# szemenyeim/RoboCupVision

Measured on AMD Instinct MI355X. Metric: training images/sec, ROBO-UNet 640x480 bs=32/GPU, higher is better.
Workload: dtype f32; 1 GPU; robo_unet_640x480_bs32; per_gpu_batch=32, global_batch=32, height=480, width=640, step=fwd+CE/argmax+bwd+L1+Adam (train.py:43-74), parallelism=dp1, launch=eager (one rcv_run per pass)

## Files before the change

robocupvision_amd/csrc/conv_bf3.hip:

```cpp
#include <type_traits>
#include "conv_bf3_stage.h"
#include "conv_epilogue.h"

constexpr int C3_PITCH = 192;
constexpr int C3_NU = 13;
constexpr int C3_COT = 64;

template <int WN, bool TWO>
__global__ __launch_bounds__(512) void conv_bf3_kernel(const ConvArgs a) {
  constexpr int WM = 2;
  extern __shared__ __attribute__((aligned(16))) char smem_c3[];
  const int npix = a.IH * a.IW;
  const int xbytes = a.xl_floats * 4;
  float* red = reinterpret_cast<float*>(smem_c3 + 2 * xbytes);
  const bool producer = threadIdx.x >= 256;
  const int tid = producer ? (int)threadIdx.x - 256 : (int)threadIdx.x;
  const TileInfo ti = decode_tile<KIND_GATHER>(a, xcd_remap(blockIdx.x, a.total_tiles), C3_COT);
  const int nchunks = a.nchunks;
  const bool do_stage = !(a.flags & RCV_F_DBG_NOSTAGE), do_mfma = !(a.flags & RCV_F_DBG_NOMFMA);

  if (producer) {
    auto stage = [&](int c, char* buf) { bf3_conv_stage<32, C3_NU, TWO>(a, ti, buf, a.Cin, 32 * c, tid, npix); };
    if (do_stage) stage(0, smem_c3);
    __syncthreads();
    for (int c = 0; c < nchunks; ++c) {
      if (c + 1 < nchunks && do_stage) stage(c + 1, smem_c3 + ((c + 1) & 1) * xbytes);
      __syncthreads();
    }
    if (a.stats != RCV_STATS_NONE) __syncthreads();
    return;
  }

  const int lane = tid & 63, wave = tid >> 6;
  const int wave_m = wave >> 1, wave_n = wave & 1;
  const int l15 = lane & 15, l4 = lane >> 4;
  f32x4 acc[WM][WN];
#pragma unroll
  for (int m = 0; m < WM; ++m)
#pragma unroll
    for (int n = 0; n < WN; ++n) acc[m][n] = (f32x4){0.f, 0.f, 0.f, 0.f};
  int pixoff[WN];
#pragma unroll
  for (int n = 0; n < WN; ++n) {
    const int p = (wave_n * WN + n) * 16 + l15;
    int ty = fd_div(p, a.fdWt), tx = p - ty * a.Wt;
    if (ty >= a.R) { ty = 0; tx = 0; }
    pixoff[n] = (ty * a.IW + tx) * C3_PITCH + l4 * 16;
  }
  const char* wb[WM];
#pragma unroll
  for (int m = 0; m < WM; ++m) {
    int co = ti.co0 + (wave_m * WM + m) * 16 + l15;
    if (co >= a.CoutP) co = a.CoutP - 1;
    wb[m] = reinterpret_cast<const char*>(a.w) + (size_t)co * 64 + l4 * 16;
  }
  const size_t wstep = (size_t)a.CoutP * 64;
  const size_t wplane = 9 * (size_t)nchunks * wstep;
  bf16x8 A[3][WM][3];
  auto load_a = [&](int tap, int c, bf16x8 (&dst)[WM][3]) {
    if (c >= nchunks) { c = nchunks - 1; }
    const size_t o = (size_t)(tap * nchunks + c) * wstep;
#pragma unroll
    for (int m = 0; m < WM; ++m)
#pragma unroll
      for (int pl = 0; pl < 3; ++pl) dst[m][pl] = *reinterpret_cast<const bf16x8*>(wb[m] + pl * wplane + o);
  };
  load_a(0, 0, A[0]);
  load_a(1, 0, A[1]);
  load_a(2, 0, A[2]);
  __syncthreads();
  for (int c = 0; c < nchunks; ++c) {
    const char* xb = smem_c3 + (c & 1) * xbytes;
    if (do_mfma)
#pragma unroll
    for (int tap = 0; tap < 9; ++tap) {
      const int tapoff = ((tap / 3) * a.IW + (tap % 3)) * C3_PITCH;
      const bf16x8 (&Ac)[WM][3] = A[tap % 3];
      bf16x8 B[2][3];
      auto load_b = [&](int n, bf16x8 (&dst)[3]) {
        const char* pb = xb + pixoff[n] + tapoff;
#pragma unroll
        for (int pl = 0; pl < 3; ++pl) dst[pl] = *reinterpret_cast<const bf16x8*>(pb + pl * 64);
      };
      load_b(0, B[0]);
#pragma unroll
      for (int n = 0; n < WN; ++n) {
        if (n + 1 < WN) load_b(n + 1, B[(n + 1) & 1]);
#pragma unroll
        for (int e = 0; e < 6; ++e)
#pragma unroll
          for (int m = 0; m < WM; ++m) acc[m][n] = __builtin_amdgcn_mfma_f32_16x16x32_bf16(Ac[m][BF3_TA[e]], B[n & 1][BF3_TB[e]], acc[m][n], 0, 0, 0);
        if (n + 1 < WN) {
#pragma unroll
          for (int e = 0; e < 3; ++e) {
            __builtin_amdgcn_sched_group_barrier(0x008, 1, 0);
            __builtin_amdgcn_sched_group_barrier(0x100, 1, 0);
          }
        }
        __builtin_amdgcn_sched_barrier(0);
      }
      {
        int t3 = tap + 3, c3 = c;
        if (t3 >= 9) { t3 -= 9; c3 += 1; }
        if (!(a.flags & RCV_F_DBG_NOSKIP)) load_a(t3, c3, A[tap % 3]);
      }
    }
    __syncthreads();
  }
  if (!(a.flags & RCV_F_DBG_NOEPI)) conv_epilogue<WM, WN, 2, 2, KIND_GATHER, 5>(a, ti, acc, red, tid);
  else if (a.stats != RCV_STATS_NONE) __syncthreads();
}

template <int WN, bool TWO>
__global__ __launch_bounds__(512) void conv2_bf3_kernel(const ConvArgs a) {
  constexpr int WM = 2, CH = 16, PITCH = 6 * CH, NKS = 5;
  extern __shared__ __attribute__((aligned(16))) char smem_c3[];
  const int npix = a.IH * a.IW;
  const int xbytes = a.xl_floats * 4;
  float* red = reinterpret_cast<float*>(smem_c3 + 2 * xbytes);
  const bool producer = threadIdx.x >= 256;
  const int tid = producer ? (int)threadIdx.x - 256 : (int)threadIdx.x;
  const TileInfo ti = decode_tile<KIND_GATHER>(a, xcd_remap(blockIdx.x, a.total_tiles), C3_COT);
  const int nchunks = a.nchunks;

  if (producer) {
    auto stage = [&](int c, char* buf) { bf3_conv_stage<CH, C3_NU, TWO>(a, ti, buf, a.Cin, CH * c, tid, npix); };
    stage(0, smem_c3);
    __syncthreads();
    for (int c = 0; c < nchunks; ++c) {
      if (c + 1 < nchunks) stage(c + 1, smem_c3 + ((c + 1) & 1) * xbytes);
      __syncthreads();
    }
    if (a.stats != RCV_STATS_NONE) __syncthreads();
// ... 93 lines not shown
    const int slots = 2 * WN * 16;
    for (int TW = 4; TW <= Wo && TW <= 64; ++TW) {
      int TH = slots / TW;
      if (TH > Ho) TH = Ho;
      if (TH < 1) continue;
      TH = ceil_div(Ho, ceil_div(Ho, TH));
      const int IH = (TH - 1) * S + 3, IW = (TW - 1) * S + 3;
      if (IH * IW > C3_NU * per_pass || IW >= 65536) continue;
      const size_t lds = 2 * (size_t)round_up(IH * IW * pitch, 16) + 2 * 2 * C3_COT * sizeof(float) * 2;
      if (lds > (size_t)h->max_lds) continue;
      const long tiles = (long)N * ceil_div(Ho, TH) * ceil_div(Wo, TW) * n_co;
      const long rounds = ceil_div((int)tiles, h->num_cus);
      const double cost = (double)rounds * (slots + 64) * (1.0 + 0.02 * (double)(IH * IW) / (TH * TW * S * S));
      if (cost < best) {
        best = cost; found = true;
        g->WN = WN; g->TH = TH; g->TW = TW; g->IH = IH; g->IW = IW; g->tiles_x = ceil_div(Wo, TW); g->tiles_y = ceil_div(Ho, TH);
        g->n_co_tiles = n_co; g->total = (int)tiles; g->lds = lds;
      }
    }
  }
  return found;
}

bool conv_bf3_wanted(const rcv_handle* h, const rcv_op* op) {
  if (RCV_ENV("RCV_NO_BF3") || (op->flags & RCV_F_MFMA_FP32)) return false;
  const int N = op->i[RCV_I_N], H = op->i[RCV_I_H], W = op->i[RCV_I_W], Cin = op->i[RCV_I_CIN], Cout = op->i[RCV_I_COUT];
  const int S = op->i[RCV_I_STRIDE];
  if (op->kind != RCV_OP_CONV || (S != 1 && S != 2) || op->i[RCV_I_DIL] != 1) return false;
  if (op->i[RCV_I_INMODE] == RCV_LOAD_NCHW || Cout % 4 || Cout < 64) return false;
  if (S == 1 ? (Cin % 32 || Cin < 64) : (Cin % 16 || Cin < 32 || RCV_ENV("RCV_NO_BF3S2") != nullptr)) return false;
  if (S == 2 && !RCV_ENV("RCV_BF3S2_ALL")) {
    const int m = op->i[RCV_I_INMODE];
    if (m == RCV_LOAD_GRAD_ENC || m == RCV_LOAD_GRAD_DEC) return false;
  }
  if ((long long)N * H * W * Cin >= (1ll << 31)) return false;
  if (RCV_ENV("RCV_BF3_FWD")) {
    const int m = op->i[RCV_I_INMODE];
    if (m == RCV_LOAD_GRAD_ENC || m == RCV_LOAD_GRAD_DEC) return false;
  }
  C3Geom g;
  if (!c3_geometry(h, op, &g)) return false;
  return (long)g.total * 4 >= (long)h->num_cus * 3;
}

bool conv_bf3_supported(const rcv_handle* h, const rcv_op* op, int kind) {
  return kind == KIND_GATHER && ((op->i[RCV_I_AUX0] == 3 && op->i[RCV_I_STRIDE] == 1) || (op->i[RCV_I_AUX0] == 5 && op->i[RCV_I_STRIDE] == 2));
}

int conv_bf3_plan(const rcv_handle* h, const rcv_op* op, ConvPlan* pl) {
  const int Cin = op->i[RCV_I_CIN], Cout = op->i[RCV_I_COUT];
  const int S = op->i[RCV_I_STRIDE];
  RCV_CHECK_ARG(op->kind == RCV_OP_CONV && (S == 1 || S == 2) && op->i[RCV_I_DIL] == 1 && Cin % (S == 1 ? 32 : 16) == 0 && Cout % 4 == 0 &&
                    op->i[RCV_I_INMODE] != RCV_LOAD_NCHW && !(op->flags & RCV_F_MFMA_FP32),
                "split-bf16 conv: needs dilation 1, Cin %% 32 == 0 (stride 1) or %% 16 (stride 2), an NHWC input (got s%d d%d Cin %d Cout %d)", S,
                op->i[RCV_I_DIL], Cin, Cout);
  C3Geom g;
  RCV_CHECK_ARG(c3_geometry(h, op, &g), "split-bf16 conv: no tile fits %dx%d", op->i[RCV_I_HO], op->i[RCV_I_WO]);
  pl->kind = KIND_GATHER; pl->narrow = 0; pl->dma = 0; pl->first = 0; pl->wino = 0; pl->small = 0; pl->bf3 = 1;
  pl->CK = S == 1 ? 32 : 16; pl->CoutV = Cout; pl->CoutP = round_up(Cout, 16);
  pl->R = g.TH; pl->Wt = g.TW; pl->IH = g.IH; pl->IW = g.IW; pl->tiles_x = g.tiles_x; pl->tiles_y = g.tiles_y;
  pl->n_co_tiles = g.n_co_tiles; pl->n_phases = 1; pl->total_tiles = g.total; pl->grid = g.total;
  pl->WN = g.WN; pl->WM = 2;
  pl->xl_floats = round_up(g.IH * g.IW * (S == 1 ? C3_PITCH : C3_PITCH / 2), 16) / 4; pl->wl_floats = 0;
  pl->lds = g.lds;
  return RCV_OK;
}

int conv_bf3_launch(const ConvPlan& pl, const ConvArgs& a, hipStream_t s) {
  const bool two = a.in_mode == RCV_LOAD_GRAD_ENC || a.in_mode == RCV_LOAD_GRAD_DEC;
  if (a.stride == 2) return two ? conv_launch_with_lds<conv2_bf3_kernel<5, true>>(pl, a, s) : conv_launch_with_lds<conv2_bf3_kernel<5, false>>(pl, a, s);
  if (pl.WN == 10) return two ? conv_launch_with_lds<conv_bf3_kernel<10, true>>(pl, a, s) : conv_launch_with_lds<conv_bf3_kernel<10, false>>(pl, a, s);
  return two ? conv_launch_with_lds<conv_bf3_kernel<5, true>>(pl, a, s) : conv_launch_with_lds<conv_bf3_kernel<5, false>>(pl, a, s);
}
```

robocupvision_amd/csrc/conv_bf3_stage.h:

```cpp
#pragma once
#include "conv_common.h"
#include "split_bf16.h"

template <int NU, bool TWO>
struct Bf3ConvRegs {
  float4 x[NU], ax[TWO ? NU : 1];
  bool ok[NU];
};

template <int CH, int NU, bool TWO>
__device__ __forceinline__ void bf3_conv_load(Bf3ConvRegs<NU, TWO>& r, const ConvArgs& a, const TileInfo& ti, int C, int c0, int tid, int npix) {
  constexpr int Q = CH / 4, PP = 256 / Q;
  const int q = tid % Q, lp = tid / Q;
#pragma unroll
  for (int u = 0; u < NU; ++u) {
    const int pix = u * PP + lp;
    const int iy = fd_div(pix, a.fdIW), ix = pix - iy * a.IW;
    const int gy = ti.oy0 + iy, gx = ti.ox0 + ix;
    r.ok[u] = pix < npix && (unsigned)gy < (unsigned)a.H && (unsigned)gx < (unsigned)a.W;
    const uint32_t o = r.ok[u] ? (uint32_t)(((ti.n * a.H + gy) * a.W + gx) * C + c0 + 4 * q) : 0u;
    r.x[u] = ld4(a.in + o);
    if (TWO) r.ax[u] = ld4(a.in_aux + o);
  }
}
template <int MODE, int CH, int NU, bool TWO>
__device__ __forceinline__ void bf3_conv_store(const Bf3ConvRegs<NU, TWO>& r, const ConvArgs& a, char* img, int C, int c0, int tid, int npix) {
  constexpr int Q = CH / 4, PP = 256 / Q;
  const int q = tid % Q, lp = tid / Q;
  float4 k[5];
  if (MODE != RCV_LOAD_PLAIN) {
#pragma unroll
    for (int j = 0; j < 5; ++j) k[j] = ld4(a.in_c + (size_t)j * C + c0 + 4 * q);
  }
#pragma unroll
  for (int u = 0; u < NU; ++u) {
    const int pix = u * PP + lp;
    float4 v = xform4<MODE>(r.x[u], r.ax[TWO ? u : 0], k);
    if (!r.ok[u]) v = make_float4(0.f, 0.f, 0.f, 0.f);
    if (pix < npix) {
      const Bf3Tri lo = bf3_split2(v.x, v.y), hi = bf3_split2(v.z, v.w);
      char* d = img + pix * (6 * CH) + 8 * q;
      *reinterpret_cast<uint2*>(d) = make_uint2(lo.h, hi.h);
      *reinterpret_cast<uint2*>(d + 2 * CH) = make_uint2(lo.m, hi.m);
      *reinterpret_cast<uint2*>(d + 4 * CH) = make_uint2(lo.l, hi.l);
    }
  }
}

template <int CH, int NU, bool TWO>
__device__ __forceinline__ void bf3_conv_stage(const ConvArgs& a, const TileInfo& ti, char* img, int C, int c0, int tid, int npix) {
  Bf3ConvRegs<NU, TWO> r;
  bf3_conv_load<CH, NU, TWO>(r, a, ti, C, c0, tid, npix);
  with_load_mode<TWO>(a.in_mode, [&](auto mode) { bf3_conv_store<mode(), CH, NU, TWO>(r, a, img, C, c0, tid, npix); });
}
```

robocupvision_amd/csrc/conv_common.h:

```cpp
#pragma once
#include "load_xform.h"

enum { KIND_GATHER = 0, KIND_TPHASE = 1, KIND_TMERGED = 2, KIND_TALL = 3 };

struct ConvArgs {
  const float* in;
  const float* in_aux;
  const float* in_c;
  const float* w;
  const float* bias;
  float* out;
  const float* resid;
  const float* epi_aux;
  const float* epi_c;
  float* part;
  int N, H, W, Cin, Cout, Ho, Wo;
  int CinP, CoutP, CoutV;
  int stride, dil;
  int R, Wt, tiles_x, tiles_y, IH, IW;
  int n_pix_tiles, n_co_tiles, n_sub, total_tiles, nchunks;
  int in_mode, stats;
  uint32_t flags;
  int wl_floats, xl_floats;
  int xpitch;
// ... 24 lines not shown
  ti.x0 = tx_i * a.Wt;
  ti.co0 = co_tile * COT;
  ti.py = phase >> 1;
  ti.px = phase & 1;
  if (KIND == KIND_GATHER) { ti.oy0 = ti.y0 * a.stride - a.dil; ti.ox0 = ti.x0 * a.stride - a.dil; }
  else { ti.oy0 = ti.y0; ti.ox0 = ti.x0; }
  return ti;
}

struct ConvPlan {
  int kind, tile, CK, R, Wt, tiles_x, tiles_y, IH, IW;
  int CoutV, CoutP, n_co_tiles, n_phases, total_tiles, grid;
  size_t lds;
  int wl_floats, xl_floats;
  int narrow;
  int dma;
  int xk;
  int WM, WN, XMAX;
  int first;
  int dev;
  int wino;
  int bf3;
  int small;
};

template <auto KERN>
static int conv_launch_with_lds(const ConvPlan& pl, const ConvArgs& a, hipStream_t s) {
  return rcv_launch_with_lds<KERN>(a, dim3(pl.grid), pl.lds, pl.dev, s);
}

static inline int conv_xpitch(int CK, int pixel_stride) {
  if (const char* ev = RCV_ENV("RCV_XPITCH_PAD")) return CK + atoi(ev);
  return pixel_stride == 1 ? CK + 2 : CK + 1;
}

static inline void tile_halo(int kind, int R, int Wt, int s, int d, int* IH, int* IW) {
  if (kind == KIND_GATHER) { *IH = (R - 1) * s + 2 * d + 1; *IW = (Wt - 1) * s + 2 * d + 1; }
  else { *IH = R + 1; *IW = Wt + 1; }
}

bool conv_wino_supported(const rcv_handle* h, const rcv_op* op, int kind);
bool conv_wino_wanted(const rcv_handle* h, const rcv_op* op, bool force);
int conv_wino_plan(const rcv_handle* h, const rcv_op* op, ConvPlan* pl);
int conv_wino_launch(const ConvPlan& pl, const ConvArgs& a, hipStream_t s);

bool conv_bf3_wanted(const rcv_handle* h, const rcv_op* op);
bool conv_bf3_supported(const rcv_handle* h, const rcv_op* op, int kind);
int conv_bf3_plan(const rcv_handle* h, const rcv_op* op, ConvPlan* pl);
int conv_bf3_launch(const ConvPlan& pl, const ConvArgs& a, hipStream_t s);

bool convn_bf3_wanted(const rcv_handle* h, const rcv_op* op);
// ... 16 lines not shown
```

robocupvision_amd/csrc/conv_epilogue.h:

```cpp
#pragma once
#include "conv_common.h"

template <int WM, int WN, int WAVES_M, int WAVES_N, int KIND, int EB = (WM == 1 ? WN : 0)>
__device__ __forceinline__ void conv_epilogue_tile(const ConvArgs& a, const TileInfo& ti, f32x4 (&acc)[WM][WN], float (&s1)[WM][4], float (&s2)[WM][4], int tid) {
  const int lane = tid & 63, wave = tid >> 6;
  const int wave_m = wave / WAVES_N, wave_n = wave % WAVES_N;
  const int l15 = lane & 15, l4 = lane >> 4;
#pragma unroll
    for (int m = 0; m < WM; ++m) {
      const int cov = ti.co0 + (wave_m * WM + m) * 16 + 4 * l4;
      int co = cov, py = ti.py, pxx = ti.px;
      if (KIND == KIND_TMERGED) { const int ph = cov / a.Cout; co = cov - ph * a.Cout; py = ph >> 1; pxx = ph & 1; }
      const bool co_ok = cov < a.CoutV;
      float4 bias = make_float4(0.f, 0.f, 0.f, 0.f);
      float4 e0 = bias, e1 = bias, mu = bias;
      if (co_ok) {
        if (a.flags & RCV_F_BIAS) bias = ld4(a.bias + co);
        if (a.stats == RCV_STATS_BWD_DEC) { e0 = ld4(a.epi_c + co); e1 = ld4(a.epi_c + a.Cout + co); }
        if (a.stats == RCV_STATS_BWD_DEC || a.stats == RCV_STATS_BWD_ENC) mu = ld4(a.epi_c + 2 * a.Cout + co);
      }
      if constexpr (EB == 0) {
#pragma unroll
        for (int b = 0; b < WN; ++b) {
          const int p = (wave_n * WN + b) * 16 + l15;
          const int ty = fd_div(p, a.fdWt), tx = p - ty * a.Wt;
          int oy = ti.y0 + ty, ox = ti.x0 + tx;
          bool ok = ty < a.R && co_ok;
          if (KIND != KIND_GATHER) {
            ok = ok && oy < a.H && ox < a.W;
            oy = 2 * oy + py; ox = 2 * ox + pxx;
// ... 50 lines not shown
              okb[i] = ok;
              offb[i] = ok ? ((size_t)(ti.n * a.Ho + oy) * a.Wo + ox) * a.Cout + co : 0;
            }
          }
          float4 rrb[EB > 0 ? EB : 1], eb[EB > 0 ? EB : 1];
          if (a.flags & RCV_F_RESID) {
  #pragma unroll
            for (int i = 0; i < EB; ++i) if (b0 + i < WN) rrb[i] = ld4(a.resid + offb[i]);
          }
          if (bwd_stats) {
  #pragma unroll
            for (int i = 0; i < EB; ++i) if (b0 + i < WN) eb[i] = ld4(a.epi_aux + offb[i]);
          }
  #pragma unroll
          for (int i = 0; i < EB; ++i) {
            const int b = b0 + i;
            if (b >= WN) continue;
            if (!okb[i]) continue;
            const size_t off = offb[i];
            float4 v = make_float4(acc[m][b][0] + bias.x, acc[m][b][1] + bias.y, acc[m][b][2] + bias.z, acc[m][b][3] + bias.w);
            if (a.flags & RCV_F_RELU) { v.x = fmaxf(v.x, 0.f); v.y = fmaxf(v.y, 0.f); v.z = fmaxf(v.z, 0.f); v.w = fmaxf(v.w, 0.f); }
            if (a.flags & RCV_F_RESID) { const float4 rr = rrb[i]; v.x += rr.x; v.y += rr.y; v.z += rr.z; v.w += rr.w; }
            *reinterpret_cast<float4*>(a.out + off) = v;
            if (a.stats == RCV_STATS_FWD) {
              s1[m][0] += v.x; s1[m][1] += v.y; s1[m][2] += v.z; s1[m][3] += v.w;
              s2[m][0] = fmaf(v.x, v.x, s2[m][0]); s2[m][1] = fmaf(v.y, v.y, s2[m][1]);
              s2[m][2] = fmaf(v.z, v.z, s2[m][2]); s2[m][3] = fmaf(v.w, v.w, s2[m][3]);
            } else if (a.stats == RCV_STATS_BWD_ENC) {
              const float4 e = eb[i];
              s1[m][0] += v.x; s1[m][1] += v.y; s1[m][2] += v.z; s1[m][3] += v.w;
              s2[m][0] = fmaf(v.x, e.x - mu.x, s2[m][0]); s2[m][1] = fmaf(v.y, e.y - mu.y, s2[m][1]);
              s2[m][2] = fmaf(v.z, e.z - mu.z, s2[m][2]); s2[m][3] = fmaf(v.w, e.w - mu.w, s2[m][3]);
            } else if (a.stats == RCV_STATS_BWD_DEC) {
              const float4 e = eb[i];
              const float gx = fmaf(e.x, e0.x, e1.x) > 0.f ? v.x : 0.f;
              const float gy = fmaf(e.y, e0.y, e1.y) > 0.f ? v.y : 0.f;
              const float gz = fmaf(e.z, e0.z, e1.z) > 0.f ? v.z : 0.f;
              const float gw = fmaf(e.w, e0.w, e1.w) > 0.f ? v.w : 0.f;
              s1[m][0] += gx; s1[m][1] += gy; s1[m][2] += gz; s1[m][3] += gw;
              s2[m][0] = fmaf(gx, e.x - mu.x, s2[m][0]); s2[m][1] = fmaf(gy, e.y - mu.y, s2[m][1]);
              s2[m][2] = fmaf(gz, e.z - mu.z, s2[m][2]); s2[m][3] = fmaf(gw, e.w - mu.w, s2[m][3]);
            }
          }
        }
      }
    }
}

template <int WM, int WAVES_M, int WAVES_N, int KIND>
__device__ __forceinline__ void conv_epilogue_stats(const ConvArgs& a, size_t row, int co0, float (&s1)[WM][4], float (&s2)[WM][4], float* red, int tid) {
  constexpr int NT = WAVES_M * WAVES_N * 64;
  constexpr int COT = WM * WAVES_M * 16;
  const int lane = tid & 63, wave = tid >> 6;
  const int wave_m = wave / WAVES_N, wave_n = wave % WAVES_N;
  const int l15 = lane & 15, l4 = lane >> 4;
    {
#pragma unroll
      for (int m = 0; m < WM; ++m)
#pragma unroll
        for (int r = 0; r < 4; ++r) {
          float u = s1[m][r], v = s2[m][r];
#pragma unroll
          for (int sh = 1; sh < 16; sh <<= 1) { u += __shfl_xor(u, sh); v += __shfl_xor(v, sh); }
          s1[m][r] = u; s2[m][r] = v;
        }
      if (l15 == 0) {
#pragma unroll
        for (int m = 0; m < WM; ++m)
#pragma unroll
          for (int r = 0; r < 4; ++r) {
            const int cl_ = (wave_m * WM + m) * 16 + 4 * l4 + r;
            red[(wave_n * 2 + 0) * COT + cl_] = s1[m][r];
            red[(wave_n * 2 + 1) * COT + cl_] = s2[m][r];
          }
      }
      __syncthreads();
      if (KIND == KIND_TMERGED) {
        for (int e = tid; e < 2 * a.Cout; e += NT) {
          const int which = e / a.Cout, co = e - which * a.Cout;
          float u = 0.f;
          for (int cv = co; cv < a.CoutV; cv += a.Cout) {
#pragma unroll
            for (int wn = 0; wn < WAVES_N; ++wn) u += red[(wn * 2 + which) * COT + cv];
          }
          a.part[(row * 2 + which) * a.Cout + co] = u;
        }
      } else {
        for (int e = tid; e < 2 * COT; e += NT) {
          const int which = e / COT, cl_ = e % COT;
          const int co = co0 + cl_;
          if (co < a.Cout) {
            float u = 0.f;
#pragma unroll
            for (int wn = 0; wn < WAVES_N; ++wn) u += red[(wn * 2 + which) * COT + cl_];
            a.part[(row * 2 + which) * a.Cout + co] = u;
          }
        }
      }
  }
}

template <int WM, int WN, int WAVES_M, int WAVES_N, int KIND, int EB = (WM == 1 ? WN : 0)>
__device__ __forceinline__ void conv_epilogue(const ConvArgs& a, const TileInfo& ti, f32x4 (&acc)[WM][WN], float* red, int tid) {
  float s1[WM][4], s2[WM][4];
#pragma unroll
  for (int m = 0; m < WM; ++m)
#pragma unroll
    for (int r = 0; r < 4; ++r) { s1[m][r] = 0.f; s2[m][r] = 0.f; }
  conv_epilogue_tile<WM, WN, WAVES_M, WAVES_N, KIND, EB>(a, ti, acc, s1, s2, tid);
  if (a.stats != RCV_STATS_NONE) {
    const size_t row = (size_t)(KIND == KIND_TPHASE ? (ti.py * 2 + ti.px) * a.n_pix_tiles : 0) + ti.pt;
    conv_epilogue_stats<WM, WAVES_M, WAVES_N, KIND>(a, row, ti.co0, s1, s2, red, tid);
  }
}
```

robocupvision_amd/csrc/rcv_internal.h:

```cpp
#pragma once
#include <hip/hip_runtime.h>
#include <stdint.h>
#include <stdio.h>
#include <stdlib.h>
#include <string.h>
#include <mutex>
#include <string>
#include <unordered_map>
#include "../../include/rcv.h"

#ifdef RCV_EXPERIMENTS
#define RCV_ENV(name) getenv(name)
#else
#define RCV_ENV(name) ((const char*)nullptr)
#endif

#define RCV_MAX_DEVICES 64

struct rcv_plan_cache {
  std::mutex mu;
  std::unordered_map<std::string, std::string> map;
};

struct rcv_handle {
// ... 62 lines not shown
  std::lock_guard<std::mutex> g(h->plans->mu);
  auto it = h->plans->map.find(rcv_plan_key(op));
  if (it == h->plans->map.end() || it->second.size() != sizeof(P)) return false;
  memcpy(out, it->second.data(), sizeof(P));
  return true;
}
template <typename P>
static inline void rcv_plan_put(const rcv_handle* h, const rcv_op* op, const P& pl) {
  if (!h->plans) return;
  std::lock_guard<std::mutex> g(h->plans->mu);
  h->plans->map[rcv_plan_key(op)] = std::string(reinterpret_cast<const char*>(&pl), sizeof(P));
}

#define RCV_ENSURE_LDS(kern, lds, dev, table)                                                                          \
  do {                                                                                                                 \
    const int d_ = ((dev) >= 0 && (dev) < RCV_MAX_DEVICES) ? (dev) : 0;                                                \
    if ((lds) > (table)[d_]) {                                                                                         \
      RCV_HIP(hipFuncSetAttribute(reinterpret_cast<const void*>(kern), hipFuncAttributeMaxDynamicSharedMemorySize, (int)(lds))); \
      (table)[d_] = (lds);                                                                                             \
    }                                                                                                                  \
  } while (0)

#if defined(__HIPCC__)
template <auto KERN, typename Args>
static int rcv_launch_with_lds(const Args& a, dim3 grid, size_t lds, int dev, hipStream_t s) {
  static size_t configured[RCV_MAX_DEVICES];
  RCV_ENSURE_LDS(KERN, lds, dev, configured);
  hipLaunchKernelGGL(KERN, grid, dim3(512), lds, s, a);
  RCV_HIP(hipGetLastError());
  return RCV_OK;
}
#endif

struct OpQuery {
  int n_part;
  int n_split;
  size_t part_bytes;
  char label[64];
};
int rcv_launch_conv(const rcv_handle* h, const rcv_op* op, hipStream_t s, OpQuery* query);
int rcv_launch_wgrad(const rcv_handle* h, const rcv_op* op, hipStream_t s, OpQuery* query);
int rcv_launch_small(const rcv_handle* h, const rcv_op* op, hipStream_t s, OpQuery* query);
int rcv_launch_pool_cls(const rcv_handle* h, const rcv_op* op, hipStream_t s, OpQuery* query);
int rcv_launch_objdet(const rcv_handle* h, const rcv_op* op, hipStream_t s, OpQuery* query);
int rcv_launch_lp_batch(const rcv_handle* h, const rcv_op* op, hipStream_t s, OpQuery* query);
int rcv_launch_lp_tail(const rcv_handle* h, const rcv_op* op, hipStream_t s, OpQuery* query);
int rcv_launch_batch_prep(const rcv_handle* h, const rcv_op* op, hipStream_t s, OpQuery* query);
int rcv_launch_cls_label(const rcv_handle* h, const rcv_op* op, hipStream_t s, OpQuery* query);
int rcv_launch_bnn(const rcv_handle* h, const rcv_op* op, hipStream_t s, OpQuery* query);
int rcv_launch_prune(const rcv_handle* h, const rcv_op* op, hipStream_t s, OpQuery* query);
int rcv_launch_objects(const rcv_handle* h, const rcv_op* op, hipStream_t s, OpQuery* query);
// ... 3 lines not shown
```

robocupvision_amd/csrc/split_bf16.h:

```cpp
#pragma once
#include "rcv_internal.h"

typedef __bf16 bf16x2 __attribute__((ext_vector_type(2)));
typedef __bf16 bf16x4 __attribute__((ext_vector_type(4)));
typedef __bf16 bf16x8 __attribute__((ext_vector_type(8)));
typedef __attribute__((address_space(3))) bf16x4 lds_bf16x4;
typedef __attribute__((address_space(3))) char lds_char;

struct Bf3Tri { uint32_t h, m, l; };
__device__ __forceinline__ uint32_t bf3_pack(float a, float b) {
  const bf16x2 v = {(__bf16)a, (__bf16)b};
  return __builtin_bit_cast(uint32_t, v);
}
__device__ __forceinline__ Bf3Tri bf3_split2(float x0, float x1) {
  Bf3Tri t;
  t.h = bf3_pack(x0, x1);
  const float r0 = x0 - __uint_as_float(t.h << 16), r1 = x1 - __uint_as_float(t.h & 0xffff0000u);
  t.m = bf3_pack(r0, r1);
  const float s0 = r0 - __uint_as_float(t.m << 16), s1 = r1 - __uint_as_float(t.m & 0xffff0000u);
  t.l = bf3_pack(s0, s1);
  return t;
}

constexpr int BF3_TA[6] = {2, 0, 1, 1, 0, 0}, BF3_TB[6] = {0, 2, 1, 0, 1, 0};

__device__ __forceinline__ bf16x8 bf3_read_tr(const lds_char* p, int off0, int off1) {
  const bf16x4 lo = __builtin_amdgcn_ds_read_tr16_b64_v4bf16((lds_bf16x4*)(p + off0));
  const bf16x4 hi = __builtin_amdgcn_ds_read_tr16_b64_v4bf16((lds_bf16x4*)(p + off1));
  return __builtin_shufflevector(lo, hi, 0, 1, 2, 3, 4, 5, 6, 7);
}
```

robocupvision_amd/csrc/wgrad_bf3.hip:

```cpp
#include "wgrad_common.h"
#include "split_bf16.h"

constexpr int B3_GPITCH = 160, B3_PPITCH = 128, B3_PPLANE = 64 * B3_PPITCH;
template <int TW>
struct B3Geom {
  static constexpr int TH = 64 / TW, IW = TW + 2, IH = TH + 2, GPIX = IH * IW;
  static constexpr int GPLANE = GPIX * B3_GPITCH;
  static constexpr int BUF = 3 * GPLANE + 3 * B3_PPLANE;
};

template <int NPIX, int TWP, bool TWO>
struct B3Regs {
  static constexpr int NU = (NPIX + 15) / 16;
  float4 x[NU], ax[TWO ? NU : 1];
  bool ok[NU];
};
template <int NPIX, int TWP, bool TWO>
__device__ __forceinline__ void b3_load(B3Regs<NPIX, TWP, TWO>& r, const float* __restrict__ src, const float* __restrict__ aux, bool two, int tid, int ch0, int C,
                                        int row0, int oy, int ox, int PH, int PW) {
  const int q = tid & 15, lp = tid >> 4;
  const int ch = ch0 + 4 * q;
#pragma unroll
  for (int u = 0; u < B3Regs<NPIX, TWP, TWO>::NU; ++u) {
    const int pix = u * 16 + lp;
// ... 11 lines not shown
  const int ch = ch0 + 4 * q;
  float4 k[5];
  if (MODE != RCV_LOAD_PLAIN) {
#pragma unroll
    for (int j = 0; j < 5; ++j) k[j] = ld4(consts + (size_t)j * C + ch);
  }
#pragma unroll
  for (int u = 0; u < B3Regs<NPIX, TWP, TWO>::NU; ++u) {
    const int pix = u * 16 + lp;
    float4 v = xform4<MODE>(r.x[u], r.ax[TWO ? u : 0], k);
    if (!r.ok[u]) v = make_float4(0.f, 0.f, 0.f, 0.f);
    if (SUM) { sum.x += v.x; sum.y += v.y; sum.z += v.z; sum.w += v.w; }
    if (pix < NPIX) {
      const Bf3Tri a = bf3_split2(v.x, v.y), b = bf3_split2(v.z, v.w);
      int off = pix * pitch + 8 * q;
      if (SWZ) off = pix * pitch + ((((q >> 2) ^ ((pix >> 1) & 3))) << 5) + 8 * (q & 3);
      *reinterpret_cast<uint2*>(img + off) = make_uint2(a.h, b.h);
      *reinterpret_cast<uint2*>(img + plane_bytes + off) = make_uint2(a.m, b.m);
      *reinterpret_cast<uint2*>(img + 2 * plane_bytes + off) = make_uint2(a.l, b.l);
    }
  }
}

template <int TW, bool GTWO>
__global__ __launch_bounds__(512) void wgrad_bf3_kernel(const WgradArgs a) {
  using G = B3Geom<TW>;
  extern __shared__ __attribute__((aligned(16))) char smem3[];
  const bool producer = threadIdx.x >= 256;
  const int tid = producer ? (int)threadIdx.x - 256 : (int)threadIdx.x;
  const int lane = tid & 63, wave = tid >> 6;
  const int wave_n = wave & 1, wave_m = wave >> 1;
  const int l15 = lane & 15, l4 = lane >> 4;

  const int n_ca_tiles = a.CAP / 64;
  const int bl = xcd_remap(blockIdx.x, gridDim.x);
  const int ctile = bl % a.nctiles, split = bl / a.nctiles;
  const int cb0 = (ctile / n_ca_tiles) * 64, ca0 = (ctile % n_ca_tiles) * 64;

  float4 bsum = make_float4(0.f, 0.f, 0.f, 0.f);
  auto stage = [&](int tile, char* buf) {
    int t = tile;
    const int tx_i = t % a.tiles_x;
    t /= a.tiles_x;
    const int ty_i = t % a.tiles_y;
    const int n = t / a.tiles_y;
    const int y0 = ty_i * G::TH, x0 = tx_i * TW;
    float4 nosum = make_float4(0.f, 0.f, 0.f, 0.f);
    B3Regs<G::GPIX, G::IW, GTWO> rg;
    B3Regs<64, TW, !GTWO> rp;
    const bool p_two = !GTWO && (a.p_mode == RCV_LOAD_GRAD_ENC || a.p_mode == RCV_LOAD_GRAD_DEC);
    b3_load(rg, a.g, a.g_aux, true, tid, ca0, a.CA, n * a.H, y0 - 1, x0 - 1, a.H, a.W);
    b3_load(rp, a.p, a.p_aux, p_two, tid, cb0, a.CB, n * a.Hp, y0, x0, a.Hp, a.Wp);
    char* gi = buf;
    char* pi = buf + 3 * G::GPLANE;
// ... 13 lines not shown
      if (producer) sb[tid] = bsum;
      __syncthreads();
      if (producer && tid < 16) {
        float4 u = make_float4(0.f, 0.f, 0.f, 0.f);
        for (int e = tid; e < 256; e += 16) { const float4 v = sb[e]; u.x += v.x; u.y += v.y; u.z += v.z; u.w += v.w; }
        *reinterpret_cast<float4*>(a.part_bias + (size_t)split * a.CBP + cb0 + 4 * tid) = u;
      }
    }
  };
  const bool do_stage = !(a.dbg & RCV_F_DBG_NOSTAGE), do_mfma = !(a.dbg & RCV_F_DBG_NOMFMA);
  if (producer) {
    if (split < a.ntiles && do_stage) stage(split, smem3);
    __syncthreads();
    int it = 0;
    for (int tile = split; tile < a.ntiles; tile += a.nsplit, ++it) {
      const int next = tile + a.nsplit;
      if (next < a.ntiles && do_stage) stage(next, smem3 + ((it + 1) & 1) * G::BUF);
      __syncthreads();
    }
    bias_partial();
    return;
  }

  f32x4 acc[9][2][2];
#pragma unroll
  for (int t = 0; t < 9; ++t)
#pragma unroll
    for (int m = 0; m < 2; ++m)
#pragma unroll
      for (int nn = 0; nn < 2; ++nn) acc[t][m][nn] = (f32x4){0.f, 0.f, 0.f, 0.f};
  const int q = l15 >> 2, p = l15 & 3;
  const int kp = 4 * l4 + q;
  int a_off[2];
#pragma unroll
  for (int m = 0; m < 2; ++m) a_off[m] = 3 * G::GPLANE + kp * B3_PPITCH + (((wave_m * 2 + m) ^ ((kp >> 1) & 3)) << 5) + 8 * p;
  const int g_row = TW == 8 ? (l4 >> 1) * G::IW + 4 * (l4 & 1) + q : kp;
  const int g_off = g_row * B3_GPITCH + (wave_n * 2) * 32 + 8 * p;
  const lds_char* lds0 = (const lds_char*)smem3;

  auto contract = [&](const lds_char* buf) {
    const lds_char* pa0 = buf + a_off[0];
    const lds_char* pa1 = buf + a_off[1];
    const lds_char* pg = buf + g_off;
#pragma unroll
    for (int j = 0; j < 2; ++j) {
      bf16x8 A[2][3];
#pragma unroll
      for (int pl = 0; pl < 3; ++pl) {
        A[0][pl] = bf3_read_tr(pa0, pl * B3_PPLANE + (32 * j) * B3_PPITCH, pl * B3_PPLANE + (32 * j + 16) * B3_PPITCH);
        A[1][pl] = bf3_read_tr(pa1, pl * B3_PPLANE + (32 * j) * B3_PPITCH, pl * B3_PPLANE + (32 * j + 16) * B3_PPITCH);
      }
      auto load_b = [&](int t, bf16x8 (&B)[2][3]) {
        const int ky = t / 3, kx = t % 3;
        const int r0 = ((TW == 8 ? 4 * j : 2 * j) + ky) * G::IW + kx;
        const int r1 = ((TW == 8 ? 4 * j + 2 : 2 * j + 1) + ky) * G::IW + kx;
#pragma unroll
        for (int pl = 0; pl < 3; ++pl)
#pragma unroll
          for (int nn = 0; nn < 2; ++nn) B[nn][pl] = bf3_read_tr(pg, pl * G::GPLANE + r0 * B3_GPITCH + nn * 32, pl * G::GPLANE + r1 * B3_GPITCH + nn * 32);
      };
      bf16x8 Bb[2][2][3];
      load_b(0, Bb[0]);
#pragma unroll
      for (int t = 0; t < 9; ++t) {
        if (t < 8) load_b(t + 1, Bb[(t + 1) & 1]);
#pragma unroll
        for (int e = 0; e < 6; ++e)
#pragma unroll
          for (int m = 0; m < 2; ++m)
#pragma unroll
            for (int nn = 0; nn < 2; ++nn) acc[t][m][nn] = __builtin_amdgcn_mfma_f32_16x16x32_bf16(A[m][BF3_TA[e]], Bb[t & 1][nn][BF3_TB[e]], acc[t][m][nn], 0, 0, 0);
        if (t < 8) {
#pragma unroll
          for (int e = 0; e < 24; ++e) {
            __builtin_amdgcn_sched_group_barrier(0x008, 1, 0);
            __builtin_amdgcn_sched_group_barrier(0x100, 1, 0);
          }
        }
        __builtin_amdgcn_sched_barrier(0);
      }
    }
  };
  __syncthreads();
  {
    int it = 0;
    for (int tile = split; tile < a.ntiles; tile += a.nsplit, ++it) {
      if (do_mfma) contract(lds0 + (it & 1) * G::BUF);
      __syncthreads();
    }
  }
  if (!(a.dbg & RCV_F_DBG_NOEPI)) {
#pragma unroll
  for (int t = 0; t < 9; ++t)
#pragma unroll
    for (int m = 0; m < 2; ++m)
#pragma unroll
      for (int nn = 0; nn < 2; ++nn)
#pragma unroll
        for (int r = 0; r < 4; ++r) {
          const int cb = cb0 + (wave_m * 2 + m) * 16 + 4 * l4 + r;
          const int ca = ca0 + (wave_n * 2 + nn) * 16 + l15;
          a.part[(((size_t)split * 9 + t) * a.CBP + cb) * a.CAP + ca] = acc[t][m][nn][r];
        }
  }
  bias_partial();
}

bool wgrad_bf3_supported(const rcv_handle* h, const rcv_op* op) {
  if (RCV_ENV("RCV_NO_BF3") || (op->flags & RCV_F_MFMA_FP32)) return false;
  const int CA = op->i[RCV_I_CIN], CB = op->i[RCV_I_COUT];
  return op->i[RCV_I_STRIDE] == 1 && op->i[RCV_I_DIL] == 1 && op->i[RCV_I_INMODE] != RCV_LOAD_NCHW && CA % 64 == 0 && CB % 64 == 0 &&
         B3Geom<16>::BUF * 2 <= h->max_lds;
}

void wgrad_bf3_geometry(const rcv_handle* h, const rcv_op* op, int* tw, int* tiles_x, int* tiles_y, int* nsplit, int* nctiles) {
  const int N = op->i[RCV_I_N], Hp = op->i[RCV_I_HO], Wp = op->i[RCV_I_WO];
  const long s8 = (long)ceil_div(Hp, 8) * ceil_div(Wp, 8), s16 = (long)ceil_div(Hp, 4) * ceil_div(Wp, 16);
  int TW = s16 < s8 ? 16 : 8;
  if (const char* ev = RCV_ENV("RCV_BF3_TW")) { const int v = atoi(ev); if (v == 8 || v == 16) TW = v; }
  *tw = TW;
  *tiles_x = ceil_div(Wp, TW); *tiles_y = ceil_div(Hp, 64 / TW);
  const int ctiles = (op->i[RCV_I_COUT] / 64) * (op->i[RCV_I_CIN] / 64);
  const int ntiles = N * *tiles_x * *tiles_y;
  int ns = h->num_cus / ctiles;
  if (ns < 1) ns = 1;
  if (ns > ntiles) ns = ntiles;
  *nsplit = ceil_div(ntiles, ceil_div(ntiles, ns));
  *nctiles = ctiles;
}

template <int TW, bool GTWO>
static int b3_launch_inst(const WgradArgs& a, dim3 grid, hipStream_t s, int dev) {
  return rcv_launch_with_lds<wgrad_bf3_kernel<TW, GTWO>>(a, grid, 2 * (size_t)B3Geom<TW>::BUF, dev, s);
}

int wgrad_bf3_launch(const rcv_handle* h, const WgradArgs& a, int tw, hipStream_t s) {
  const bool g_two = a.g_mode == RCV_LOAD_GRAD_ENC || a.g_mode == RCV_LOAD_GRAD_DEC;
  const dim3 grid(a.nsplit * a.nctiles);
  if (tw == 8) return g_two ? b3_launch_inst<8, true>(a, grid, s, h->device) : b3_launch_inst<8, false>(a, grid, s, h->device);
  return g_two ? b3_launch_inst<16, true>(a, grid, s, h->device) : b3_launch_inst<16, false>(a, grid, s, h->device);
}
```

Measured before the change: 5916 img/s.

## Split bf3 conv consumer work across four wave columns with chained stats epilogue

Adds a 768-thread variant of the split-bf16 3x3 conv kernel in which 8 consumer waves (4 along N) each hold half the accumulators (WN=5 instead of 10), used for stride-1 forward/dgrad tiles that previously ran WN=10. A chained epilogue lets paired wave columns pass BN statistics partials through LDS, and a lean staging mode shrinks address registers. The wgrad kernel gains the same 4-column template, but it is only selected when 'w' is in the two-consumer list, which by default holds just 'f' and 'd'. The intent is lower register pressure and more MFMA-issuing waves per block, at the cost of extra LDS traffic and barriers in the epilogue.

```diff
diff --git a/robocupvision_amd/csrc/conv_bf3.hip b/robocupvision_amd/csrc/conv_bf3.hip
--- a/robocupvision_amd/csrc/conv_bf3.hip
+++ b/robocupvision_amd/csrc/conv_bf3.hip
@@ -6,33 +6,37 @@
 constexpr int C3_NU = 13;
 constexpr int C3_COT = 64;
 
-template <int WN, bool TWO>
-__global__ __launch_bounds__(512) void conv_bf3_kernel(const ConvArgs a) {
-  constexpr int WM = 2;
+template <int WN, bool TWO, int WAVES_N = 2>
+__global__ __launch_bounds__(128 * WAVES_N + 256) void conv_bf3_kernel(const ConvArgs a) {
+  constexpr int WM = 2, NC = 128 * WAVES_N;
+  constexpr bool LEAN = WAVES_N == 4;
   extern __shared__ __attribute__((aligned(16))) char smem_c3[];
   const int npix = a.IH * a.IW;
   const int xbytes = a.xl_floats * 4;
   float* red = reinterpret_cast<float*>(smem_c3 + 2 * xbytes);
-  const bool producer = threadIdx.x >= 256;
-  const int tid = producer ? (int)threadIdx.x - 256 : (int)threadIdx.x;
+  const bool producer = threadIdx.x >= NC;
+  const int tid = producer ? (int)threadIdx.x - NC : (int)threadIdx.x;
   const TileInfo ti = decode_tile<KIND_GATHER>(a, xcd_remap(blockIdx.x, a.total_tiles), C3_COT);
   const int nchunks = a.nchunks;
   const bool do_stage = !(a.flags & RCV_F_DBG_NOSTAGE), do_mfma = !(a.flags & RCV_F_DBG_NOMFMA);
 
   if (producer) {
-    auto stage = [&](int c, char* buf) { bf3_conv_stage<32, C3_NU, TWO>(a, ti, buf, a.Cin, 32 * c, tid, npix); };
+    auto stage = [&](int c, char* buf) { bf3_conv_stage<32, C3_NU, TWO, LEAN>(a, ti, buf, a.Cin, 32 * c, tid, npix); };
     if (do_stage) stage(0, smem_c3);
     __syncthreads();
     for (int c = 0; c < nchunks; ++c) {
       if (c + 1 < nchunks && do_stage) stage(c + 1, smem_c3 + ((c + 1) & 1) * xbytes);
       __syncthreads();
     }
-    if (a.stats != RCV_STATS_NONE) __syncthreads();
+    if (a.stats != RCV_STATS_NONE) {
+      __syncthreads();
+      if (WAVES_N == 4) __syncthreads();
+    }
     return;
   }
 
   const int lane = tid & 63, wave = tid >> 6;
-  const int wave_m = wave >> 1, wave_n = wave & 1;
+  const int wave_m = wave >> (WAVES_N == 4 ? 2 : 1), wave_n = wave & (WAVES_N - 1);
   const int l15 = lane & 15, l4 = lane >> 4;
   f32x4 acc[WM][WN];
 #pragma unroll
@@ -47,12 +51,14 @@
     if (ty >= a.R) { ty = 0; tx = 0; }
     pixoff[n] = (ty * a.IW + tx) * C3_PITCH + l4 * 16;
   }
-  const char* wb[WM];
+  const char* wu = reinterpret_cast<const char*>(a.w);
+  std::conditional_t<LEAN, uint32_t, const char*> wb[WM];
 #pragma unroll
   for (int m = 0; m < WM; ++m) {
     int co = ti.co0 + (wave_m * WM + m) * 16 + l15;
     if (co >= a.CoutP) co = a.CoutP - 1;
-    wb[m] = reinterpret_cast<const char*>(a.w) + (size_t)co * 64 + l4 * 16;
+    if constexpr (LEAN) wb[m] = (uint32_t)(co * 64 + l4 * 16);
+    else wb[m] = wu + (size_t)co * 64 + l4 * 16;
   }
   const size_t wstep = (size_t)a.CoutP * 64;
   const size_t wplane = 9 * (size_t)nchunks * wstep;
@@ -63,7 +69,10 @@
 #pragma unroll
     for (int m = 0; m < WM; ++m)
 #pragma unroll
-      for (int pl = 0; pl < 3; ++pl) dst[m][pl] = *reinterpret_cast<const bf16x8*>(wb[m] + pl * wplane + o);
+      for (int pl = 0; pl < 3; ++pl) {
+        if constexpr (LEAN) dst[m][pl] = *reinterpret_cast<const bf16x8*>(wu + (pl * wplane + o) + wb[m]);
+        else dst[m][pl] = *reinterpret_cast<const bf16x8*>(wb[m] + pl * wplane + o);
+      }
   };
   load_a(0, 0, A[0]);
   load_a(1, 0, A[1]);
@@ -107,8 +116,13 @@
     }
     __syncthreads();
   }
-  if (!(a.flags & RCV_F_DBG_NOEPI)) conv_epilogue<WM, WN, 2, 2, KIND_GATHER, 5>(a, ti, acc, red, tid);
-  else if (a.stats != RCV_STATS_NONE) __syncthreads();
+  if (!(a.flags & RCV_F_DBG_NOEPI)) {
+    if constexpr (WAVES_N == 4) conv_epilogue_chained<WM, WN, 2, 4, KIND_GATHER, 5>(a, ti, acc, red, reinterpret_cast<float*>(smem_c3), tid);
+    else conv_epilogue<WM, WN, 2, WAVES_N, KIND_GATHER, 5>(a, ti, acc, red, tid);
+  } else if (a.stats != RCV_STATS_NONE) {
+    __syncthreads();
+    if (WAVES_N == 4) __syncthreads();
+  }
 }
 
 template <int WN, bool TWO>
@@ -248,6 +262,8 @@
   return found;
 }
 
+static bool conv_is_dgrad(const rcv_op* op) { return op->i[RCV_I_INMODE] == RCV_LOAD_GRAD_ENC || op->i[RCV_I_INMODE] == RCV_LOAD_GRAD_DEC; }
+
 bool conv_bf3_wanted(const rcv_handle* h, const rcv_op* op) {
   if (RCV_ENV("RCV_NO_BF3") || (op->flags & RCV_F_MFMA_FP32)) return false;
   const int N = op->i[RCV_I_N], H = op->i[RCV_I_H], W = op->i[RCV_I_W], Cin = op->i[RCV_I_CIN], Cout = op->i[RCV_I_COUT];
@@ -287,6 +303,7 @@
   pl->R = g.TH; pl->Wt = g.TW; pl->IH = g.IH; pl->IW = g.IW; pl->tiles_x = g.tiles_x; pl->tiles_y = g.tiles_y;
   pl->n_co_tiles = g.n_co_tiles; pl->n_phases = 1; pl->total_tiles = g.total; pl->grid = g.total;
   pl->WN = g.WN; pl->WM = 2;
+  pl->waves_n = g.WN == 10 && S == 1 && bf3_two_consumers(conv_is_dgrad(op) ? 'd' : 'f') ? 4 : 2;
   pl->xl_floats = round_up(g.IH * g.IW * (S == 1 ? C3_PITCH : C3_PITCH / 2), 16) / 4; pl->wl_floats = 0;
   pl->lds = g.lds;
   return RCV_OK;
@@ -295,6 +312,8 @@
 int conv_bf3_launch(const ConvPlan& pl, const ConvArgs& a, hipStream_t s) {
   const bool two = a.in_mode == RCV_LOAD_GRAD_ENC || a.in_mode == RCV_LOAD_GRAD_DEC;
   if (a.stride == 2) return two ? conv_launch_with_lds<conv2_bf3_kernel<5, true>>(pl, a, s) : conv_launch_with_lds<conv2_bf3_kernel<5, false>>(pl, a, s);
+  if (pl.WN == 10 && pl.waves_n == 4)
+    return two ? conv_launch_with_lds<conv_bf3_kernel<5, true, 4>, 768>(pl, a, s) : conv_launch_with_lds<conv_bf3_kernel<5, false, 4>, 768>(pl, a, s);
   if (pl.WN == 10) return two ? conv_launch_with_lds<conv_bf3_kernel<10, true>>(pl, a, s) : conv_launch_with_lds<conv_bf3_kernel<10, false>>(pl, a, s);
   return two ? conv_launch_with_lds<conv_bf3_kernel<5, true>>(pl, a, s) : conv_launch_with_lds<conv_bf3_kernel<5, false>>(pl, a, s);
 }
diff --git a/robocupvision_amd/csrc/conv_bf3_stage.h b/robocupvision_amd/csrc/conv_bf3_stage.h
--- a/robocupvision_amd/csrc/conv_bf3_stage.h
+++ b/robocupvision_amd/csrc/conv_bf3_stage.h
@@ -23,7 +23,7 @@
     if (TWO) r.ax[u] = ld4(a.in_aux + o);
   }
 }
-template <int MODE, int CH, int NU, bool TWO>
+template <int MODE, int CH, int NU, bool TWO, bool LEAN = false>
 __device__ __forceinline__ void bf3_conv_store(const Bf3ConvRegs<NU, TWO>& r, const ConvArgs& a, char* img, int C, int c0, int tid, int npix) {
   constexpr int Q = CH / 4, PP = 256 / Q;
   const int q = tid % Q, lp = tid / Q;
@@ -39,7 +39,7 @@
     if (!r.ok[u]) v = make_float4(0.f, 0.f, 0.f, 0.f);
     if (pix < npix) {
       const Bf3Tri lo = bf3_split2(v.x, v.y), hi = bf3_split2(v.z, v.w);
-      char* d = img + pix * (6 * CH) + 8 * q;
+      char* d = LEAN ? img + lp * (6 * CH) + 8 * q + u * (PP * 6 * CH) : img + pix * (6 * CH) + 8 * q;
       *reinterpret_cast<uint2*>(d) = make_uint2(lo.h, hi.h);
       *reinterpret_cast<uint2*>(d + 2 * CH) = make_uint2(lo.m, hi.m);
       *reinterpret_cast<uint2*>(d + 4 * CH) = make_uint2(lo.l, hi.l);
@@ -47,9 +47,9 @@
   }
 }
 
-template <int CH, int NU, bool TWO>
+template <int CH, int NU, bool TWO, bool LEAN = false>
 __device__ __forceinline__ void bf3_conv_stage(const ConvArgs& a, const TileInfo& ti, char* img, int C, int c0, int tid, int npix) {
   Bf3ConvRegs<NU, TWO> r;
   bf3_conv_load<CH, NU, TWO>(r, a, ti, C, c0, tid, npix);
-  with_load_mode<TWO>(a.in_mode, [&](auto mode) { bf3_conv_store<mode(), CH, NU, TWO>(r, a, img, C, c0, tid, npix); });
+  with_load_mode<TWO>(a.in_mode, [&](auto mode) { bf3_conv_store<mode(), CH, NU, TWO, LEAN>(r, a, img, C, c0, tid, npix); });
 }
diff --git a/robocupvision_amd/csrc/conv_common.h b/robocupvision_amd/csrc/conv_common.h
--- a/robocupvision_amd/csrc/conv_common.h
+++ b/robocupvision_amd/csrc/conv_common.h
@@ -70,11 +70,12 @@
   int wino;
   int bf3;
   int small;
+  int waves_n;
 };
 
-template <auto KERN>
+template <auto KERN, int THREADS = 512>
 static int conv_launch_with_lds(const ConvPlan& pl, const ConvArgs& a, hipStream_t s) {
-  return rcv_launch_with_lds<KERN>(a, dim3(pl.grid), pl.lds, pl.dev, s);
+  return rcv_launch_with_lds<KERN, THREADS>(a, dim3(pl.grid), pl.lds, pl.dev, s);
 }
 
 static inline int conv_xpitch(int CK, int pixel_stride) {
diff --git a/robocupvision_amd/csrc/conv_epilogue.h b/robocupvision_amd/csrc/conv_epilogue.h
--- a/robocupvision_amd/csrc/conv_epilogue.h
+++ b/robocupvision_amd/csrc/conv_epilogue.h
@@ -1,11 +1,14 @@
 #pragma once
 #include "conv_common.h"
 
-template <int WM, int WN, int WAVES_M, int WAVES_N, int KIND, int EB = (WM == 1 ? WN : 0)>
-__device__ __forceinline__ void conv_epilogue_tile(const ConvArgs& a, const TileInfo& ti, f32x4 (&acc)[WM][WN], float (&s1)[WM][4], float (&s2)[WM][4], int tid) {
+template <int WM, int WN, int WAVES_M, int WAVES_N, int KIND, int EB = (WM == 1 ? WN : 0), bool CHAIN = false>
+__device__ __forceinline__ void conv_epilogue_tile(const ConvArgs& a, const TileInfo& ti, f32x4 (&acc)[WM][WN], float (&s1)[WM][4], float (&s2)[WM][4], int tid,
+                                                   f32x4* dd = nullptr, uint32_t* okm = nullptr) {
+  static_assert(!CHAIN || EB > 0, "the chained form is written for the batched epilogue");
   const int lane = tid & 63, wave = tid >> 6;
   const int wave_m = wave / WAVES_N, wave_n = wave % WAVES_N;
   const int l15 = lane & 15, l4 = lane >> 4;
+  const bool defer = CHAIN && (wave_n & 1) && a.stats != RCV_STATS_NONE;
 #pragma unroll
     for (int m = 0; m < WM; ++m) {
       const int cov = ti.co0 + (wave_m * WM + m) * 16 + 4 * l4;
@@ -102,6 +105,23 @@
             if (a.flags & RCV_F_RELU) { v.x = fmaxf(v.x, 0.f); v.y = fmaxf(v.y, 0.f); v.z = fmaxf(v.z, 0.f); v.w = fmaxf(v.w, 0.f); }
             if (a.flags & RCV_F_RESID) { const float4 rr = rrb[i]; v.x += rr.x; v.y += rr.y; v.z += rr.z; v.w += rr.w; }
             *reinterpret_cast<float4*>(a.out + off) = v;
+            if constexpr (CHAIN) {
+              if (defer) {
+                float4 t = v, f = v;
+                if (bwd_stats) {
+                  const float4 e = eb[i];
+                  f = make_float4(e.x - mu.x, e.y - mu.y, e.z - mu.z, e.w - mu.w);
+                  if (a.stats == RCV_STATS_BWD_DEC) {
+                    t.x = fmaf(e.x, e0.x, e1.x) > 0.f ? v.x : 0.f; t.y = fmaf(e.y, e0.y, e1.y) > 0.f ? v.y : 0.f;
+                    t.z = fmaf(e.z, e0.z, e1.z) > 0.f ? v.z : 0.f; t.w = fmaf(e.w, e0.w, e1.w) > 0.f ? v.w : 0.f;
+                  }
+                }
+                acc[m][b] = (f32x4){t.x, t.y, t.z, t.w};
+                dd[m * WN + b] = (f32x4){f.x, f.y, f.z, f.w};
+                *okm |= 1u << (m * WN + b);
+                continue;
+              }
+            }
             if (a.stats == RCV_STATS_FWD) {
               s1[m][0] += v.x; s1[m][1] += v.y; s1[m][2] += v.z; s1[m][3] += v.w;
               s2[m][0] = fmaf(v.x, v.x, s2[m][0]); s2[m][1] = fmaf(v.y, v.y, s2[m][1]);
@@ -128,13 +148,15 @@
 }
 
 template <int WM, int WAVES_M, int WAVES_N, int KIND>
-__device__ __forceinline__ void conv_epilogue_stats(const ConvArgs& a, size_t row, int co0, float (&s1)[WM][4], float (&s2)[WM][4], float* red, int tid) {
+__device__ __forceinline__ void conv_epilogue_stats(const ConvArgs& a, size_t row, int co0, float (&s1)[WM][4], float (&s2)[WM][4], float* red, int tid,
+                                                    bool active = true) {
   constexpr int NT = WAVES_M * WAVES_N * 64;
   constexpr int COT = WM * WAVES_M * 16;
   const int lane = tid & 63, wave = tid >> 6;
   const int wave_m = wave / WAVES_N, wave_n = wave % WAVES_N;
   const int l15 = lane & 15, l4 = lane >> 4;
     {
+      if (active) {
 #pragma unroll
       for (int m = 0; m < WM; ++m)
 #pragma unroll
@@ -154,7 +176,9 @@
             red[(wave_n * 2 + 1) * COT + cl_] = s2[m][r];
           }
       }
+      }
       __syncthreads();
+      if (!active) return;
       if (KIND == KIND_TMERGED) {
         for (int e = tid; e < 2 * a.Cout; e += NT) {
           const int which = e / a.Cout, co = e - which * a.Cout;
@@ -193,3 +217,44 @@
     conv_epilogue_stats<WM, WAVES_M, WAVES_N, KIND>(a, row, ti.co0, s1, s2, red, tid);
   }
 }
+
+template <int WM, int WN, int WAVES_M, int WAVES_N, int KIND, int EB>
+__device__ __forceinline__ void conv_epilogue_chained(const ConvArgs& a, const TileInfo& ti, f32x4 (&acc)[WM][WN], float* red, float* chain, int tid) {
+  static_assert(WAVES_N % 2 == 0 && WM * WN <= 32, "pairs of wave columns; one bit per accumulator block");
+  float s1[WM][4], s2[WM][4];
+#pragma unroll
+  for (int m = 0; m < WM; ++m)
+#pragma unroll
+    for (int r = 0; r < 4; ++r) { s1[m][r] = 0.f; s2[m][r] = 0.f; }
+  f32x4 dd[WM * WN];
+  uint32_t okm = 0;
+  conv_epilogue_tile<WM, WN, WAVES_M, WAVES_N, KIND, EB, true>(a, ti, acc, s1, s2, tid, dd, &okm);
+  if (a.stats == RCV_STATS_NONE) return;
+  const int lane = tid & 63, wave = tid >> 6;
+  const int wave_m = wave / WAVES_N, wave_n = wave % WAVES_N;
+  const bool second = wave_n & 1;
+  const int pair = wave_m * (WAVES_N / 2) + (wave_n >> 1);
+  float* ch = chain + pair * (WM * 8 * 64) + lane;
+  if (!second) {
+#pragma unroll
+    for (int m = 0; m < WM; ++m)
+#pragma unroll
+      for (int r = 0; r < 4; ++r) { ch[(m * 8 + r) * 64] = s1[m][r]; ch[(m * 8 + 4 + r) * 64] = s2[m][r]; }
+  }
+  __syncthreads();
+  if (second) {
+#pragma unroll
+    for (int m = 0; m < WM; ++m) {
+#pragma unroll
+      for (int r = 0; r < 4; ++r) { s1[m][r] = ch[(m * 8 + r) * 64]; s2[m][r] = ch[(m * 8 + 4 + r) * 64]; }
+#pragma unroll
+      for (int b = 0; b < WN; ++b) {
+        if (!((okm >> (m * WN + b)) & 1u)) continue;
+#pragma unroll
+        for (int r = 0; r < 4; ++r) { s1[m][r] += acc[m][b][r]; s2[m][r] = fmaf(acc[m][b][r], dd[m * WN + b][r], s2[m][r]); }
+      }
+    }
+  }
+  const size_t row = (size_t)(KIND == KIND_TPHASE ? (ti.py * 2 + ti.px) * a.n_pix_tiles : 0) + ti.pt;
+  conv_epilogue_stats<WM, WAVES_M, WAVES_N / 2, KIND>(a, row, ti.co0, s1, s2, red, pair * 64 + lane, second);
+}
diff --git a/robocupvision_amd/csrc/rcv_internal.h b/robocupvision_amd/csrc/rcv_internal.h
--- a/robocupvision_amd/csrc/rcv_internal.h
+++ b/robocupvision_amd/csrc/rcv_internal.h
@@ -108,11 +108,11 @@
   } while (0)
 
 #if defined(__HIPCC__)
-template <auto KERN, typename Args>
+template <auto KERN, int THREADS = 512, typename Args>
 static int rcv_launch_with_lds(const Args& a, dim3 grid, size_t lds, int dev, hipStream_t s) {
   static size_t configured[RCV_MAX_DEVICES];
   RCV_ENSURE_LDS(KERN, lds, dev, configured);
-  hipLaunchKernelGGL(KERN, grid, dim3(512), lds, s, a);
+  hipLaunchKernelGGL(KERN, grid, dim3(THREADS), lds, s, a);
   RCV_HIP(hipGetLastError());
   return RCV_OK;
 }
diff --git a/robocupvision_amd/csrc/split_bf16.h b/robocupvision_amd/csrc/split_bf16.h
--- a/robocupvision_amd/csrc/split_bf16.h
+++ b/robocupvision_amd/csrc/split_bf16.h
@@ -29,3 +29,9 @@
   const bf16x4 hi = __builtin_amdgcn_ds_read_tr16_b64_v4bf16((lds_bf16x4*)(p + off1));
   return __builtin_shufflevector(lo, hi, 0, 1, 2, 3, 4, 5, 6, 7);
 }
+
+constexpr const char* BF3_TWO_CONSUMERS = "fd";
+static inline bool bf3_two_consumers(char dir) {
+  if (const char* ev = RCV_ENV("RCV_BF3_ONEC")) return strchr(ev, dir) == nullptr;
+  return strchr(BF3_TWO_CONSUMERS, dir) != nullptr;
+}
diff --git a/robocupvision_amd/csrc/wgrad_bf3.hip b/robocupvision_amd/csrc/wgrad_bf3.hip
--- a/robocupvision_amd/csrc/wgrad_bf3.hip
+++ b/robocupvision_amd/csrc/wgrad_bf3.hip
@@ -57,14 +57,15 @@
   }
 }
 
-template <int TW, bool GTWO>
-__global__ __launch_bounds__(512) void wgrad_bf3_kernel(const WgradArgs a) {
+template <int TW, bool GTWO, int WAVES_N = 2>
+__global__ __launch_bounds__(128 * WAVES_N + 256) void wgrad_bf3_kernel(const WgradArgs a) {
   using G = B3Geom<TW>;
+  constexpr int NC = 128 * WAVES_N, NN = 4 / WAVES_N;
   extern __shared__ __attribute__((aligned(16))) char smem3[];
-  const bool producer = threadIdx.x >= 256;
-  const int tid = producer ? (int)threadIdx.x - 256 : (int)threadIdx.x;
+  const bool producer = threadIdx.x >= NC;
+  const int tid = producer ? (int)threadIdx.x - NC : (int)threadIdx.x;
   const int lane = tid & 63, wave = tid >> 6;
-  const int wave_n = wave & 1, wave_m = wave >> 1;
+  const int wave_n = wave & (WAVES_N - 1), wave_m = wave >> (WAVES_N == 4 ? 2 : 1);
   const int l15 = lane & 15, l4 = lane >> 4;
 
   const int n_ca_tiles = a.CAP / 64;
@@ -124,20 +125,20 @@
     return;
   }
 
-  f32x4 acc[9][2][2];
+  f32x4 acc[9][2][NN];
 #pragma unroll
   for (int t = 0; t < 9; ++t)
 #pragma unroll
     for (int m = 0; m < 2; ++m)
 #pragma unroll
-      for (int nn = 0; nn < 2; ++nn) acc[t][m][nn] = (f32x4){0.f, 0.f, 0.f, 0.f};
+      for (int nn = 0; nn < NN; ++nn) acc[t][m][nn] = (f32x4){0.f, 0.f, 0.f, 0.f};
   const int q = l15 >> 2, p = l15 & 3;
   const int kp = 4 * l4 + q;
   int a_off[2];
 #pragma unroll
   for (int m = 0; m < 2; ++m) a_off[m] = 3 * G::GPLANE + kp * B3_PPITCH + (((wave_m * 2 + m) ^ ((kp >> 1) & 3)) << 5) + 8 * p;
   const int g_row = TW == 8 ? (l4 >> 1) * G::IW + 4 * (l4 & 1) + q : kp;
-  const int g_off = g_row * B3_GPITCH + (wave_n * 2) * 32 + 8 * p;
+  const int g_off = g_row * B3_GPITCH + (wave_n * NN) * 32 + 8 * p;
   const lds_char* lds0 = (const lds_char*)smem3;
 
   auto contract = [&](const lds_char* buf) {
@@ -152,16 +153,16 @@
         A[0][pl] = bf3_read_tr(pa0, pl * B3_PPLANE + (32 * j) * B3_PPITCH, pl * B3_PPLANE + (32 * j + 16) * B3_PPITCH);
         A[1][pl] = bf3_read_tr(pa1, pl * B3_PPLANE + (32 * j) * B3_PPITCH, pl * B3_PPLANE + (32 * j + 16) * B3_PPITCH);
       }
-      auto load_b = [&](int t, bf16x8 (&B)[2][3]) {
+      auto load_b = [&](int t, bf16x8 (&B)[NN][3]) {
         const int ky = t / 3, kx = t % 3;
         const int r0 = ((TW == 8 ? 4 * j : 2 * j) + ky) * G::IW + kx;
         const int r1 = ((TW == 8 ? 4 * j + 2 : 2 * j + 1) + ky) * G::IW + kx;
 #pragma unroll
         for (int pl = 0; pl < 3; ++pl)
 #pragma unroll
-          for (int nn = 0; nn < 2; ++nn) B[nn][pl] = bf3_read_tr(pg, pl * G::GPLANE + r0 * B3_GPITCH + nn * 32, pl * G::GPLANE + r1 * B3_GPITCH + nn * 32);
+          for (int nn = 0; nn < NN; ++nn) B[nn][pl] = bf3_read_tr(pg, pl * G::GPLANE + r0 * B3_GPITCH + nn * 32, pl * G::GPLANE + r1 * B3_GPITCH + nn * 32);
       };
-      bf16x8 Bb[2][2][3];
+      bf16x8 Bb[2][NN][3];
       load_b(0, Bb[0]);
 #pragma unroll
       for (int t = 0; t < 9; ++t) {
@@ -171,10 +172,10 @@
 #pragma unroll
           for (int m = 0; m < 2; ++m)
 #pragma unroll
-            for (int nn = 0; nn < 2; ++nn) acc[t][m][nn] = __builtin_amdgcn_mfma_f32_16x16x32_bf16(A[m][BF3_TA[e]], Bb[t & 1][nn][BF3_TB[e]], acc[t][m][nn], 0, 0, 0);
+            for (int nn = 0; nn < NN; ++nn) acc[t][m][nn] = __builtin_amdgcn_mfma_f32_16x16x32_bf16(A[m][BF3_TA[e]], Bb[t & 1][nn][BF3_TB[e]], acc[t][m][nn], 0, 0, 0);
         if (t < 8) {
 #pragma unroll
-          for (int e = 0; e < 24; ++e) {
+          for (int e = 0; e < 12 * NN; ++e) {
             __builtin_amdgcn_sched_group_barrier(0x008, 1, 0);
             __builtin_amdgcn_sched_group_barrier(0x100, 1, 0);
           }
@@ -197,11 +198,11 @@
 #pragma unroll
     for (int m = 0; m < 2; ++m)
 #pragma unroll
-      for (int nn = 0; nn < 2; ++nn)
+      for (int nn = 0; nn < NN; ++nn)
 #pragma unroll
         for (int r = 0; r < 4; ++r) {
           const int cb = cb0 + (wave_m * 2 + m) * 16 + 4 * l4 + r;
-          const int ca = ca0 + (wave_n * 2 + nn) * 16 + l15;
+          const int ca = ca0 + (wave_n * NN + nn) * 16 + l15;
           a.part[(((size_t)split * 9 + t) * a.CBP + cb) * a.CAP + ca] = acc[t][m][nn][r];
         }
   }
@@ -233,7 +234,8 @@
 
 template <int TW, bool GTWO>
 static int b3_launch_inst(const WgradArgs& a, dim3 grid, hipStream_t s, int dev) {
-  return rcv_launch_with_lds<wgrad_bf3_kernel<TW, GTWO>>(a, grid, 2 * (size_t)B3Geom<TW>::BUF, dev, s);
+  if (bf3_two_consumers('w')) return rcv_launch_with_lds<wgrad_bf3_kernel<TW, GTWO, 4>, 768>(a, grid, 2 * (size_t)B3Geom<TW>::BUF, dev, s);
+  return rcv_launch_with_lds<wgrad_bf3_kernel<TW, GTWO, 2>, 512>(a, grid, 2 * (size_t)B3Geom<TW>::BUF, dev, s);
 }
 
 int wgrad_bf3_launch(const rcv_handle* h, const WgradArgs& a, int tw, hipStream_t s) {
```

Result: no change. 5948 img/s (median of 4 runs) (+0.6%).
